# henriChevreux/distillation_trajectories

Measured on AMD Instinct MI355X. Metric: trajectory-timesteps/sec (B×T U-Net fwd) at 16×16 T=50, higher is better.
Workload: dtype f32 (fp32-accurate; convolutions: exact 3-plane bf16 operand split on bf16 MFMA with fp32 accumulate, or native fp32 MFMA, chosen per layer)

## Files before the change

### distillation_trajectories_amd/csrc/dt_conv_strip.hip

```cpp
#include <mutex>
#include <type_traits>

#include "dt_conv_epilogue.h"

namespace dt {

extern __shared__ __attribute__((aligned(16))) __bf16 strip_lds[];

template <int BM, int BN, int KC, int WK>
__global__ __launch_bounds__(256, find_strip_form(BM, BN, KC, WK)->waves_per_simd()) void conv_strip_bf16x6_kernel(const ConvParams p) {
  constexpr ConvForm F = *find_strip_form(BM, BN, KC, WK);
  constexpr int WN = F.wn(), WM = F.wm(), NT = 256;
  constexpr int MI = F.mi(), NI = F.ni();
  constexpr int KW = F.kw();
  static_assert(WM * WN * WK * 64 == NT && KC % WK == 0 && MI * 32 * WM == BM && NI * 32 * WN == BN && (WK == 1 || (MI == 2 && NI == 2)), "wave layout");
  constexpr int PLANE_B = F.plane_b(), STAGE_B = 3 * PLANE_B;
  constexpr int AP = F.ap();
  static_assert(2 * (BM + 2 * (F.max_w() + 1)) <= AP * NT, "strip staging reach");
  const int halo = strip_halo(p.W, BM);
  const int R = F.strip_rows(halo);
  const int RZ = F.zero_row(R);
  const int PLANE_A = F.plane_a(RZ);
  __bf16 *As = strip_lds;
  __bf16 *Bs = strip_lds + F.strip_elems(PLANE_A);

  const int tid = threadIdx.x, lane = tid & 63;
  const int wave = __builtin_amdgcn_readfirstlane(tid >> 6);
  const int wk = wave % WK, wm = (wave / WK) / WN, wn = (wave / WK) % WN;
  const int half = lane >> 5, l31 = lane & 31;
  const int m0 = blockIdx.x * BM, n0 = blockIdx.y * BN;
  const int HW = p.H * p.W;
  const int CC = p.cin_p >> 4;

  bool s_in[AP], s_ok[AP], s_core[AP];
  int s_off[AP], s_off2[AP], s_offb[AP], s_lds[AP];
#pragma unroll
  for (int i = 0; i < AP; ++i) {
    const int item = tid + i * NT;
    const int srow = item >> 1, hh = item & 1;
    const int m = m0 - halo + srow;
    s_in[i] = item < 2 * R;
    s_ok[i] = s_in[i] && m >= 0 && m < p.M;
    s_core[i] = s_ok[i] && srow >= halo && srow < halo + BM;
    const int mm = s_ok[i] ? m : 0;
    s_off[i] = mm * p.cin_p + hh * 8;
    s_off2[i] = mm * p.cin2_p + hh * 8;
    s_offb[i] = mm * p.b_stride + hh * 8;
    s_lds[i] = srow * 16 + ((hh ^ ((srow >> 3) & 1)) << 3);
  }
  constexpr bool B_ALL = WK > 1 && BN * 4 == NT;
  constexpr int NB = B_ALL ? KC * 3 / 2 : KC * 3, SB = B_ALL ? 2 : 1;
  static_assert(!B_ALL || (KC * 3) % 2 == 0, "weight staging");
  const bool b_thread = B_ALL || tid < BN * 2;
  const int bt = B_ALL ? (tid & (BN * 2 - 1)) : tid, bsub = B_ALL ? tid / (BN * 2) : 0;
  const size_t w_plane = (size_t)p.n_p * 16;
  const __bf16 *wbase = reinterpret_cast<const __bf16 *>(p.w) + (size_t)n0 * 16 + bt * 8 + bsub * w_plane;
  const __bf16 *wbase2 = reinterpret_cast<const __bf16 *>(p.w2) + (size_t)n0 * 16 + bt * 8 + bsub * w_plane;
  const int b_lds = bsub * PLANE_B + bt * 8;

  int a_row[MI];
  unsigned a_mask[MI];
#pragma unroll
  for (int mi = 0; mi < MI; ++mi) {
    const int row_i = wm * (MI * 32) + mi * 32 + l31;
    const int m = m0 + row_i;
    a_row[mi] = row_i + halo;
    unsigned mask = 0;
    if (m < p.M) {
      const int rem = m % HW;
      const int y = rem / p.W, x = rem - y * p.W;
#pragma unroll
      for (int t = 0; t < 9; ++t) {
        const int yy = y + t / 3 - 1, xx = x + t % 3 - 1;
        if (yy >= 0 && yy < p.H && xx >= 0 && xx < p.W) mask |= 1u << t;
      }
    }
    a_mask[mi] = mask;
  }
  int b_frag[NI];
#pragma unroll
  for (int ni = 0; ni < NI; ++ni) {
    const int row = wn * (NI * 32) + ni * 32 + l31;
    b_frag[ni] = row * 16 + ((half ^ ((row >> 3) & 1)) << 3);
  }

  f32x16 acc[MI][NI];
#pragma unroll
  for (int mi = 0; mi < MI; ++mi)
#pragma unroll
    for (int ni = 0; ni < NI; ++ni)
#pragma unroll
      for (int r = 0; r < 16; ++r) acc[mi][ni][r] = 0.f;

  const int n_main = (CC + p.splits * KC - 1) / (p.splits * KC);
  const int cc0 = blockIdx.z * n_main * KC;
  const int CC2 = p.cin2_p >> 4;
  const int n_chunks = n_main + (p.in2 ? (CC2 + KC - 1) / KC : 0);

  f32x4 sa0[KC][AP], sa1[KC][AP];
  u32x4 rb[NB];
  auto load_strip = [&](int ch) __attribute__((always_inline)) {
#pragma unroll
    for (int kk = 0; kk < KC; ++kk)
#pragma unroll
    for (int i = 0; i < AP; ++i) {
      sa0[kk][i] = f32x4{0.f, 0.f, 0.f, 0.f}; sa1[kk][i] = sa0[kk][i];
      if (ch < n_main) {
        const int cc = cc0 + ch * KC + kk;
        if (s_ok[i] && cc < CC) {
          const float *src = (p.in_b && cc >= p.cc_a) ? p.in_b + s_offb[i] + (cc - p.cc_a) * 16 : p.in + s_off[i] + cc * 16;
          sa0[kk][i] = *reinterpret_cast<const f32x4 *>(src);
          sa1[kk][i] = *reinterpret_cast<const f32x4 *>(src + 4);
        }
      } else if (s_core[i] && (ch - n_main) * KC + kk < CC2) {
        const int c2 = (ch - n_main) * KC + kk;
        const float *src = (p.in2_b && c2 >= p.cc_a) ? p.in2_b + s_offb[i] + (c2 - p.cc_a) * 16 : p.in2 + s_off2[i] + c2 * 16;
        sa0[kk][i] = *reinterpret_cast<const f32x4 *>(src);
        sa1[kk][i] = *reinterpret_cast<const f32x4 *>(src + 4);
      }
    }
  };
  auto write_strip = [&]() __attribute__((always_inline)) {
#pragma unroll
    for (int kk = 0; kk < KC; ++kk)
#pragma unroll
    for (int i = 0; i < AP; ++i)
      if (s_in[i]) {
        bf16x8 p1, p2, p3;
        split8(sa0[kk][i], sa1[kk][i], p1, p2, p3);
        __bf16 *A = As + kk * 3 * PLANE_A;
        *reinterpret_cast<bf16x8 *>(A + s_lds[i]) = p1;
        *reinterpret_cast<bf16x8 *>(A + PLANE_A + s_lds[i]) = p2;
        *reinterpret_cast<bf16x8 *>(A + 2 * PLANE_A + s_lds[i]) = p3;
      }
  };
  const size_t tap_stride = (size_t)p.ccw * 3 * w_plane, group_stride = (size_t)KC * 3 * w_plane;
  const __bf16 *wrun = wbase + (size_t)cc0 * 3 * w_plane;
  enum { ADV_NONE = 0, ADV_TAP, ADV_GROUP, ADV_SKIP0, ADV_SKIP };
  auto load_b = [&](int adv) __attribute__((always_inline)) {
    if (adv == ADV_TAP) wrun += tap_stride;
    else if (adv == ADV_GROUP) wrun = wrun - 8 * tap_stride + group_stride;
    else if (adv == ADV_SKIP0) wrun = wbase2;
    else if (adv == ADV_SKIP) wrun += group_stride;
    if (b_thread) {
#pragma unroll
      for (int i = 0; i < NB; ++i)
        rb[i] = *reinterpret_cast<const u32x4 *>(wrun + (SB * i) * w_plane);
    }
  };
  auto write_b = [&](int stage) __attribute__((always_inline)) {
    if (b_thread) {
      __bf16 *B = Bs + stage * KC * STAGE_B;
#pragma unroll
      for (int i = 0; i < NB; ++i) *reinterpret_cast<u32x4 *>(B + (SB * i) * PLANE_B + b_lds) = rb[i];
    }
  };

  constexpr bool DB = WK > 1;
  bf16x8 fbn[KW][NI][3];
  auto load_bd = [&](int adv) __attribute__((always_inline)) {
    if (adv == ADV_TAP) wrun += tap_stride;
    else if (adv == ADV_GROUP) wrun = wrun - 8 * tap_stride + group_stride;
    else if (adv == ADV_SKIP0) wrun = wbase2;
    else if (adv == ADV_SKIP) wrun += group_stride;
    const __bf16 *wt = wrun - (bt * 8 + bsub * w_plane);
#pragma unroll
    for (int kw = 0; kw < KW; ++kw)
#pragma unroll
      for (int ni = 0; ni < NI; ++ni)
#pragma unroll
        for (int pl = 0; pl < 3; ++pl)
          fbn[kw][ni][pl] = *reinterpret_cast<const bf16x8 *>(wt + ((wk * KW + kw) * 3 + pl) * w_plane + b_frag[ni]);
  };

  load_strip(0);
  if (DB) load_bd(ADV_NONE); else load_b(ADV_NONE);
  if (tid < 48 * KC) *reinterpret_cast<u32x4 *>(As + (tid >> 4) * PLANE_A + RZ * 16 + (tid & 15) * 8) = u32x4{0u, 0u, 0u, 0u};
  write_strip();
  if (!DB) write_b(0);
  __syncthreads();

  int step = 0;
  bool stage_next_strip = true;
  auto do_step = [&](auto TT, int ch, bool first_tap, bool last_tap, bool next_chunk, int adv) __attribute__((always_inline)) {
    constexpr int tt = decltype(TT)::value;
    const bool more = !last_tap || next_chunk;
    if (first_tap && next_chunk && stage_next_strip) load_strip(ch + 1);
    bf16x8 fbc[KW][NI][3];
    if (DB) {
#pragma unroll
      for (int kw = 0; kw < KW; ++kw)
#pragma unroll
        for (int ni = 0; ni < NI; ++ni)
#pragma unroll
          for (int pl = 0; pl < 3; ++pl) fbc[kw][ni][pl] = fbn[kw][ni][pl];
      if (more) load_bd(adv);
    } else if (more) load_b(adv);
    {
      int wv = p.W;
      asm volatile("" : "+s"(wv));
      const int shift = (tt / 3 - 1) * wv + (tt % 3 - 1);
      int a_e[MI];
#pragma unroll
      for (int mi = 0; mi < MI; ++mi) {
        int row0 = a_row[mi];
        asm volatile("" : "+v"(row0));
        const int srow = row0 + shift;
        const int lrow = ((a_mask[mi] >> tt) & 1u) ? srow : RZ + (srow & 7);
        a_e[mi] = lrow * 16 + ((half ^ ((srow >> 3) & 1)) << 3);
      }
#pragma unroll
      for (int kw = 0; kw < KW; ++kw) {
        const int kk = wk * KW + kw;
        const __bf16 *A = As + kk * 3 * PLANE_A;
        const __bf16 *B = Bs + ((step & 1) * KC + kk) * STAGE_B;
        bf16x8 fb[NI][3];
#pragma unroll
        for (int ni = 0; ni < NI; ++ni)
#pragma unroll
          for (int pl = 0; pl < 3; ++pl)
            fb[ni][pl] = DB ? fbc[kw][ni][pl] : *reinterpret_cast<const bf16x8 *>(B + pl * PLANE_B + b_frag[ni]);
#pragma unroll
        for (int mi = 0; mi < MI; ++mi) {
          bf16x8 fa[3];
#pragma unroll
          for (int pl = 0; pl < 3; ++pl)
            fa[pl] = *reinterpret_cast<const bf16x8 *>(A + pl * PLANE_A + a_e[mi]);
#pragma unroll
          for (int ni = 0; ni < NI; ++ni) mfma_bf16x6(acc[mi][ni], fa, fb[ni]);
        }
      }
    }
    if (!DB && more) write_b((step + 1) & 1);
    const bool restage = last_tap && next_chunk && stage_next_strip;
    if (restage) {
      __syncthreads();
      write_strip();
    }
    if (!DB || restage) __syncthreads();
    ++step;
  };

  constexpr bool DIRECT = MI * KW <= 2 && KC >= 2;
  f32x4 ga0[KW][MI][2], ga1[KW][MI][2];
  const int n_skip = p.in2 ? (CC2 + KC - 1) / KC : 0;
  auto load_a = [&](f32x4 (&g)[KW][MI][2], int s2) __attribute__((always_inline)) {
#pragma unroll
    for (int kw = 0; kw < KW; ++kw)
#pragma unroll
      for (int mi = 0; mi < MI; ++mi) {
        const int c2 = s2 * KC + wk * KW + kw;
        const int m = m0 + wm * (MI * 32) + mi * 32 + l31;
        g[kw][mi][0] = f32x4{0.f, 0.f, 0.f, 0.f}; g[kw][mi][1] = g[kw][mi][0];
        if (m < p.M && c2 < CC2) {
          const float *src = (p.in2_b && c2 >= p.cc_a) ? p.in2_b + (size_t)m * p.b_stride + (c2 - p.cc_a) * 16 + half * 8
                                                       : p.in2 + (size_t)m * p.cin2_p + c2 * 16 + half * 8;
          g[kw][mi][0] = *reinterpret_cast<const f32x4 *>(src);
          g[kw][mi][1] = *reinterpret_cast<const f32x4 *>(src + 4);
        }
      }
  };
  auto skip_step = [&](f32x4 (&g)[KW][MI][2], int s2) __attribute__((always_inline)) {
    const bool more = s2 + 1 < n_skip;
    bf16x8 fbc[KW][NI][3];
    if (DB) {
#pragma unroll
      for (int kw = 0; kw < KW; ++kw)
#pragma unroll
        for (int ni = 0; ni < NI; ++ni)
#pragma unroll
          for (int pl = 0; pl < 3; ++pl) fbc[kw][ni][pl] = fbn[kw][ni][pl];
      if (more) load_bd(ADV_SKIP);
    } else if (more) load_b(ADV_SKIP);
#pragma unroll
    for (int kw = 0; kw < KW; ++kw) {
      const int kk = wk * KW + kw;
      const __bf16 *B = Bs + ((step & 1) * KC + kk) * STAGE_B;
      bf16x8 fb[NI][3];
#pragma unroll
      for (int ni = 0; ni < NI; ++ni)
#pragma unroll
        for (int pl = 0; pl < 3; ++pl) fb[ni][pl] = DB ? fbc[kw][ni][pl] : *reinterpret_cast<const bf16x8 *>(B + pl * PLANE_B + b_frag[ni]);
#pragma unroll
      for (int mi = 0; mi < MI; ++mi) {
        bf16x8 fa[3];
        split8(g[kw][mi][0], g[kw][mi][1], fa[0], fa[1], fa[2]);
#pragma unroll
        for (int ni = 0; ni < NI; ++ni) mfma_bf16x6(acc[mi][ni], fa, fb[ni]);
      }
    }
    if (s2 + 2 < n_skip) load_a(g, s2 + 2);
    if (!DB) {
      if (more) write_b((step + 1) & 1);
      __syncthreads();
    }
    ++step;
  };

  const int prio_grp = ((blockIdx.x + gridDim.x * (blockIdx.y + gridDim.y * blockIdx.z)) >> 8) & 1;
  const bool use_prio = gridDim.x * gridDim.y * gridDim.z <= 512;
  for (int ch = 0; ch < n_main; ++ch) {
    if (use_prio) {
      if ((ch ^ prio_grp) & 1) __builtin_amdgcn_s_setprio(1);
      else __builtin_amdgcn_s_setprio(0);
    }
    const bool next_chunk = ch + 1 < ((WK > 1 && p.in2) ? n_main : n_chunks);
    if (DIRECT && WK == 1 && p.in2 && ch + 1 == n_main) {
      stage_next_strip = false;
      load_a(ga0, 0);
      if (n_skip > 1) load_a(ga1, 1);
    }
    do_step(std::integral_constant<int, 0>{}, ch, true, false, next_chunk, ADV_TAP);
    do_step(std::integral_constant<int, 1>{}, ch, false, false, next_chunk, ADV_TAP);
    do_step(std::integral_constant<int, 2>{}, ch, false, false, next_chunk, ADV_TAP);
    do_step(std::integral_constant<int, 3>{}, ch, false, false, next_chunk, ADV_TAP);
    do_step(std::integral_constant<int, 4>{}, ch, false, false, next_chunk, ADV_TAP);
    do_step(std::integral_constant<int, 5>{}, ch, false, false, next_chunk, ADV_TAP);
    do_step(std::integral_constant<int, 6>{}, ch, false, false, next_chunk, ADV_TAP);
    do_step(std::integral_constant<int, 7>{}, ch, false, false, next_chunk, ADV_TAP);
    do_step(std::integral_constant<int, 8>{}, ch, false, true, next_chunk, ch + 1 < n_main ? ADV_GROUP : ADV_SKIP0);
    if constexpr (WK == 1) {
      if (ch + 1 == n_main && p.in2) conv_midpoint<MI, NI>(p, acc, n0, wn, l31);
    }
  }
  if constexpr (WK > 1) {
    if (p.in2) {
      constexpr int P = F.pitch(), COPY = F.copy_floats();
      float *red = reinterpret_cast<float *>(strip_lds);
#pragma unroll
      for (int mi = 0; mi < MI; ++mi) {
        if (mi || DB) __syncthreads();
#pragma unroll
        for (int ni = 0; ni < NI; ++ni)
#pragma unroll
          for (int r = 0; r < 16; ++r)
            red[wk * COPY + (wm * 32 + 4 * half + (r & 3) + 8 * (r >> 2)) * P + wn * (NI * 32) + ni * 32 + l31] = acc[mi][ni][r];
        __syncthreads();
#pragma unroll
        for (int ni = 0; ni < NI; ++ni)
#pragma unroll
          for (int r = 0; r < 16; ++r) {
            const float *src = red + (wm * 32 + 4 * half + (r & 3) + 8 * (r >> 2)) * P + wn * (NI * 32) + ni * 32 + l31;
            float v = src[0];
#pragma unroll
            for (int c = 1; c < WK; ++c) v += src[c * COPY];
            acc[mi][ni][r] = wk == 0 ? v : 0.f;
          }
      }
      if (wk == 0) conv_midpoint<MI, NI>(p, acc, n0, wn, l31);
      __syncthreads();
      if (DB) load_bd(ADV_SKIP0); else load_b(ADV_SKIP0);
      if (DIRECT) {
        load_a(ga0, 0);
        if (n_skip > 1) load_a(ga1, 1);
      } else {
        load_strip(n_main);
        if (tid < 48 * KC) *reinterpret_cast<u32x4 *>(As + (tid >> 4) * PLANE_A + RZ * 16 + (tid & 15) * 8) = u32x4{0u, 0u, 0u, 0u};
        write_strip();
      }
      if (!DB) write_b(step & 1);
      __syncthreads();
    }
  }
  __builtin_amdgcn_s_setprio(0);
  if (DIRECT) {
    for (int s2 = 0; s2 < n_skip; s2 += 2) {
      skip_step(ga0, s2);
      if (s2 + 1 < n_skip) skip_step(ga1, s2 + 1);
    }
  } else {
    for (int ch = n_main; ch < n_chunks; ++ch)
      do_step(std::integral_constant<int, 4>{}, ch, true, true, ch + 1 < n_chunks, ADV_SKIP);
  }
  conv_epilogue<BM, BN, WK>(p, acc, reinterpret_cast<float *>(strip_lds), m0, n0, wm, wn, half, l31, wk);
}

#define DT_STRIP_ROW(cls, kind, bm, bn, kc, wk) {{kind, bm, bn, kc, wk, cls}, conv_strip_bf16x6_kernel<bm, bn, kc, wk>},
static const ConvKernel kStripKernels[] = {DT_CONV_FORMS_ALL_STRIP(DT_STRIP_ROW)};

static int strip_lds_attribute() {
  constexpr int kMaxDevices = 64;
  static std::mutex mu;
  static int status[kMaxDevices];
  int dev = 0;
  DT_HIP_TRY(hipGetDevice(&dev));
  if (dev < 0 || dev >= kMaxDevices) return DT_E_ARG;
  std::lock_guard<std::mutex> lock(mu);
  if (status[dev] == 0) {
    status[dev] = 1;
    for (const ConvKernel &k : kStripKernels) {
      if (!k.form.needs_lds_attribute()) continue;
      const hipError_t e = hipFuncSetAttribute(reinterpret_cast<const void *>(k.fn), hipFuncAttributeMaxDynamicSharedMemorySize, (int)k.form.lds_limit());
      if (e != hipSuccess) status[dev] = -(int)e;
    }
  }
  return status[dev] == 1 ? DT_OK : -status[dev];
}

int launch_conv_strip(const ConvParams &p_in, hipStream_t s) {
  ConvParams p = p_in;
  const ConvKernel &k = conv_kernel_of(kStripKernels, p);
  size_t lds = k.form.lds_bytes(p.W);
  p.dup_stage2 = p.n_dup == 2 && p.pool_out && k.form.dup_stage_bytes() <= k.form.lds_limit();
  if (p.dup_stage2 && k.form.dup_stage_bytes() > lds) lds = k.form.dup_stage_bytes();
  if (const int st = k.form.needs_lds_attribute() ? strip_lds_attribute() : DT_OK) return st;
  k.fn<<<dim3((p.M + p.bm - 1) / p.bm, p.n_p / p.bn, p.splits), 256, lds, s>>>(p);
  DT_LAUNCH_CHECK();
  return DT_OK;
}

}
```

Before: 349,000.

## Slim strip-kernel staging state and defer skip-input params to kernarg reload

Replaces the per-slot arrays of flags and three precomputed offsets with a single clamped row index plus an LDS slot that is -1 for inactive slots. Main and skip inputs become descriptor structs passed to one generic strip loader. The final main chunk is peeled out of the loop so the skip-path handling no longer needs runtime branches inside it. Skip-input parameters and the second weight base are re-read from the kernarg segment only after the main loop, to shorten their live ranges and cut register pressure. In exchange, offsets are recomputed with a multiply on every load, and skip strips now also load halo rows that are never used.

```diff
diff --git a/distillation_trajectories_amd/csrc/dt_conv_strip.hip b/distillation_trajectories_amd/csrc/dt_conv_strip.hip
--- a/distillation_trajectories_amd/csrc/dt_conv_strip.hip
+++ b/distillation_trajectories_amd/csrc/dt_conv_strip.hip
@@ -32,21 +32,15 @@
   const int HW = p.H * p.W;
   const int CC = p.cin_p >> 4;
 
-  bool s_in[AP], s_ok[AP], s_core[AP];
-  int s_off[AP], s_off2[AP], s_offb[AP], s_lds[AP];
+  const int s_h8 = (tid & 1) * 8;
+  int s_m[AP], s_lds[AP];
 #pragma unroll
   for (int i = 0; i < AP; ++i) {
     const int item = tid + i * NT;
     const int srow = item >> 1, hh = item & 1;
     const int m = m0 - halo + srow;
-    s_in[i] = item < 2 * R;
-    s_ok[i] = s_in[i] && m >= 0 && m < p.M;
-    s_core[i] = s_ok[i] && srow >= halo && srow < halo + BM;
-    const int mm = s_ok[i] ? m : 0;
-    s_off[i] = mm * p.cin_p + hh * 8;
-    s_off2[i] = mm * p.cin2_p + hh * 8;
-    s_offb[i] = mm * p.b_stride + hh * 8;
-    s_lds[i] = srow * 16 + ((hh ^ ((srow >> 3) & 1)) << 3);
+    s_m[i] = (item < 2 * R && m >= 0 && m < p.M) ? m : 0;
+    s_lds[i] = item < 2 * R ? srow * 16 + ((hh ^ ((srow >> 3) & 1)) << 3) : -1;
   }
   constexpr bool B_ALL = WK > 1 && BN * 4 == NT;
   constexpr int NB = B_ALL ? KC * 3 / 2 : KC * 3, SB = B_ALL ? 2 : 1;
@@ -55,7 +49,7 @@
   const int bt = B_ALL ? (tid & (BN * 2 - 1)) : tid, bsub = B_ALL ? tid / (BN * 2) : 0;
   const size_t w_plane = (size_t)p.n_p * 16;
   const __bf16 *wbase = reinterpret_cast<const __bf16 *>(p.w) + (size_t)n0 * 16 + bt * 8 + bsub * w_plane;
-  const __bf16 *wbase2 = reinterpret_cast<const __bf16 *>(p.w2) + (size_t)n0 * 16 + bt * 8 + bsub * w_plane;
+  const __bf16 *wbase2 = nullptr;
   const int b_lds = bsub * PLANE_B + bt * 8;
 
   int a_row[MI];
@@ -94,45 +88,49 @@
 
   const int n_main = (CC + p.splits * KC - 1) / (p.splits * KC);
   const int cc0 = blockIdx.z * n_main * KC;
-  const int CC2 = p.cin2_p >> 4;
-  const int n_chunks = n_main + (p.in2 ? (CC2 + KC - 1) / KC : 0);
+  const bool has_skip = p.in2 != nullptr;
+
+  struct StripSrc { const float *a, *b; int stride_a, stride_b, cc_split, cc_n; };
+  const StripSrc main_src = {p.in, p.in_b, p.cin_p, p.b_stride, p.in_b ? p.cc_a : CC, CC};
+  StripSrc skip_src = {};
 
   f32x4 sa0[KC][AP], sa1[KC][AP];
   u32x4 rb[NB];
-  auto load_strip = [&](int ch) __attribute__((always_inline)) {
+  auto load_strip = [&](const StripSrc &src, int c0) __attribute__((always_inline)) {
+#pragma unroll
+    for (int kk = 0; kk < KC; ++kk) {
+      const int cc = c0 + kk;
+      const bool live = cc < src.cc_n;
+      const bool from_b = cc >= src.cc_split;
+      const float *base = from_b ? src.b + (cc - src.cc_split) * 16 : src.a + cc * 16;
+      const int stride = from_b ? src.stride_b : src.stride_a;
+#pragma unroll
+      for (int i = 0; i < AP; ++i) {
+        sa0[kk][i] = f32x4{0.f, 0.f, 0.f, 0.f}; sa1[kk][i] = sa0[kk][i];
+        if (live) {
+          const float *s = base + (s_m[i] * stride + s_h8);
+          sa0[kk][i] = *reinterpret_cast<const f32x4 *>(s);
+          sa1[kk][i] = *reinterpret_cast<const f32x4 *>(s + 4);
+        }
+      }
+    }
+  };
+  auto write_strip = [&]() __attribute__((always_inline)) {
 #pragma unroll
     for (int kk = 0; kk < KC; ++kk)
 #pragma unroll
     for (int i = 0; i < AP; ++i) {
-      sa0[kk][i] = f32x4{0.f, 0.f, 0.f, 0.f}; sa1[kk][i] = sa0[kk][i];
-      if (ch < n_main) {
-        const int cc = cc0 + ch * KC + kk;
-        if (s_ok[i] && cc < CC) {
-          const float *src = (p.in_b && cc >= p.cc_a) ? p.in_b + s_offb[i] + (cc - p.cc_a) * 16 : p.in + s_off[i] + cc * 16;
-          sa0[kk][i] = *reinterpret_cast<const f32x4 *>(src);
-          sa1[kk][i] = *reinterpret_cast<const f32x4 *>(src + 4);
-        }
-      } else if (s_core[i] && (ch - n_main) * KC + kk < CC2) {
-        const int c2 = (ch - n_main) * KC + kk;
-        const float *src = (p.in2_b && c2 >= p.cc_a) ? p.in2_b + s_offb[i] + (c2 - p.cc_a) * 16 : p.in2 + s_off2[i] + c2 * 16;
-        sa0[kk][i] = *reinterpret_cast<const f32x4 *>(src);
-        sa1[kk][i] = *reinterpret_cast<const f32x4 *>(src + 4);
-      }
-    }
-  };
-  auto write_strip = [&]() __attribute__((always_inline)) {
-#pragma unroll
-    for (int kk = 0; kk < KC; ++kk)
-#pragma unroll
-    for (int i = 0; i < AP; ++i)
-      if (s_in[i]) {
+      int slot = s_lds[i];
+      asm volatile("" : "+v"(slot));
+      if (slot >= 0) {
         bf16x8 p1, p2, p3;
         split8(sa0[kk][i], sa1[kk][i], p1, p2, p3);
         __bf16 *A = As + kk * 3 * PLANE_A;
-        *reinterpret_cast<bf16x8 *>(A + s_lds[i]) = p1;
-        *reinterpret_cast<bf16x8 *>(A + PLANE_A + s_lds[i]) = p2;
-        *reinterpret_cast<bf16x8 *>(A + 2 * PLANE_A + s_lds[i]) = p3;
-      }
+        *reinterpret_cast<bf16x8 *>(A + slot) = p1;
+        *reinterpret_cast<bf16x8 *>(A + PLANE_A + slot) = p2;
+        *reinterpret_cast<bf16x8 *>(A + 2 * PLANE_A + slot) = p3;
+      }
+    }
   };
   const size_t tap_stride = (size_t)p.ccw * 3 * w_plane, group_stride = (size_t)KC * 3 * w_plane;
   const __bf16 *wrun = wbase + (size_t)cc0 * 3 * w_plane;
@@ -173,7 +171,7 @@
           fbn[kw][ni][pl] = *reinterpret_cast<const bf16x8 *>(wt + ((wk * KW + kw) * 3 + pl) * w_plane + b_frag[ni]);
   };
 
-  load_strip(0);
+  load_strip(main_src, cc0);
   if (DB) load_bd(ADV_NONE); else load_b(ADV_NONE);
   if (tid < 48 * KC) *reinterpret_cast<u32x4 *>(As + (tid >> 4) * PLANE_A + RZ * 16 + (tid & 15) * 8) = u32x4{0u, 0u, 0u, 0u};
   write_strip();
@@ -181,11 +179,11 @@
   __syncthreads();
 
   int step = 0;
-  bool stage_next_strip = true;
-  auto do_step = [&](auto TT, int ch, bool first_tap, bool last_tap, bool next_chunk, int adv) __attribute__((always_inline)) {
+  auto do_step = [&](auto TT, bool first_tap, bool last_tap, bool next_chunk, int adv, const StripSrc &next, int c_next,
+                     bool stage_next) __attribute__((always_inline)) {
     constexpr int tt = decltype(TT)::value;
     const bool more = !last_tap || next_chunk;
-    if (first_tap && next_chunk && stage_next_strip) load_strip(ch + 1);
+    if (first_tap && next_chunk && stage_next) load_strip(next, c_next);
     bf16x8 fbc[KW][NI][3];
     if (DB) {
 #pragma unroll
@@ -232,7 +230,7 @@
       }
     }
     if (!DB && more) write_b((step + 1) & 1);
-    const bool restage = last_tap && next_chunk && stage_next_strip;
+    const bool restage = last_tap && next_chunk && stage_next;
     if (restage) {
       __syncthreads();
       write_strip();
@@ -241,9 +239,43 @@
     ++step;
   };
 
+  const int prio_grp = ((blockIdx.x + gridDim.x * (blockIdx.y + gridDim.y * blockIdx.z)) >> 8) & 1;
+  const bool use_prio = gridDim.x * gridDim.y * gridDim.z <= 512;
+  auto chunk_group = [&](int ch, bool next_chunk, int adv_last, const StripSrc &next, int c_next, bool stage_next) __attribute__((always_inline)) {
+    if (use_prio) {
+      if ((ch ^ prio_grp) & 1) __builtin_amdgcn_s_setprio(1);
+      else __builtin_amdgcn_s_setprio(0);
+    }
+    do_step(std::integral_constant<int, 0>{}, true, false, next_chunk, ADV_TAP, next, c_next, stage_next);
+    do_step(std::integral_constant<int, 1>{}, false, false, next_chunk, ADV_TAP, next, c_next, stage_next);
+    do_step(std::integral_constant<int, 2>{}, false, false, next_chunk, ADV_TAP, next, c_next, stage_next);
+    do_step(std::integral_constant<int, 3>{}, false, false, next_chunk, ADV_TAP, next, c_next, stage_next);
+    do_step(std::integral_constant<int, 4>{}, false, false, next_chunk, ADV_TAP, next, c_next, stage_next);
+    do_step(std::integral_constant<int, 5>{}, false, false, next_chunk, ADV_TAP, next, c_next, stage_next);
+    do_step(std::integral_constant<int, 6>{}, false, false, next_chunk, ADV_TAP, next, c_next, stage_next);
+    do_step(std::integral_constant<int, 7>{}, false, false, next_chunk, ADV_TAP, next, c_next, stage_next);
+    do_step(std::integral_constant<int, 8>{}, false, true, next_chunk, adv_last, next, c_next, stage_next);
+  };
+  const int n_loop = (WK == 1 && has_skip) ? n_main - 1 : n_main;
+  for (int ch = 0; ch < n_loop; ++ch)
+    chunk_group(ch, ch + 1 < n_main, ADV_GROUP, main_src, cc0 + (ch + 1) * KC, true);
+
+  typedef const __attribute__((address_space(4))) ConvParams KernargParams;
+  KernargParams *qp = (KernargParams *)__builtin_amdgcn_kernarg_segment_ptr();
+  asm volatile("" : "+s"(qp));
+  const ConvParams q = *(const ConvParams *)qp;
+
   constexpr bool DIRECT = MI * KW <= 2 && KC >= 2;
   f32x4 ga0[KW][MI][2], ga1[KW][MI][2];
-  const int n_skip = p.in2 ? (CC2 + KC - 1) / KC : 0;
+  int n_skip = 0;
+  if (has_skip) {
+    const int CC2 = q.cin2_p >> 4;
+    skip_src = StripSrc{q.in2, q.in2_b, q.cin2_p, q.b_stride, q.in2_b ? q.cc_a : CC2, CC2};
+    n_skip = (CC2 + KC - 1) / KC;
+    wbase2 = reinterpret_cast<const __bf16 *>(q.w2) + (size_t)n0 * 16 + bt * 8 + bsub * w_plane;
+  }
+  const int n_chunks = n_main + n_skip;
+  const int M_rows = q.M;
   auto load_a = [&](f32x4 (&g)[KW][MI][2], int s2) __attribute__((always_inline)) {
 #pragma unroll
     for (int kw = 0; kw < KW; ++kw)
@@ -252,9 +284,9 @@
         const int c2 = s2 * KC + wk * KW + kw;
         const int m = m0 + wm * (MI * 32) + mi * 32 + l31;
         g[kw][mi][0] = f32x4{0.f, 0.f, 0.f, 0.f}; g[kw][mi][1] = g[kw][mi][0];
-        if (m < p.M && c2 < CC2) {
-          const float *src = (p.in2_b && c2 >= p.cc_a) ? p.in2_b + (size_t)m * p.b_stride + (c2 - p.cc_a) * 16 + half * 8
-                                                       : p.in2 + (size_t)m * p.cin2_p + c2 * 16 + half * 8;
+        if (m < M_rows && c2 < skip_src.cc_n) {
+          const float *src = c2 >= skip_src.cc_split ? skip_src.b + (size_t)m * skip_src.stride_b + (c2 - skip_src.cc_split) * 16 + half * 8
+                                                     : skip_src.a + (size_t)m * skip_src.stride_a + c2 * 16 + half * 8;
           g[kw][mi][0] = *reinterpret_cast<const f32x4 *>(src);
           g[kw][mi][1] = *reinterpret_cast<const f32x4 *>(src + 4);
         }
@@ -297,34 +329,18 @@
     ++step;
   };
 
-  const int prio_grp = ((blockIdx.x + gridDim.x * (blockIdx.y + gridDim.y * blockIdx.z)) >> 8) & 1;
-  const bool use_prio = gridDim.x * gridDim.y * gridDim.z <= 512;
-  for (int ch = 0; ch < n_main; ++ch) {
-    if (use_prio) {
-      if ((ch ^ prio_grp) & 1) __builtin_amdgcn_s_setprio(1);
-      else __builtin_amdgcn_s_setprio(0);
-    }
-    const bool next_chunk = ch + 1 < ((WK > 1 && p.in2) ? n_main : n_chunks);
-    if (DIRECT && WK == 1 && p.in2 && ch + 1 == n_main) {
-      stage_next_strip = false;
-      load_a(ga0, 0);
-      if (n_skip > 1) load_a(ga1, 1);
-    }
-    do_step(std::integral_constant<int, 0>{}, ch, true, false, next_chunk, ADV_TAP);
-    do_step(std::integral_constant<int, 1>{}, ch, false, false, next_chunk, ADV_TAP);
-    do_step(std::integral_constant<int, 2>{}, ch, false, false, next_chunk, ADV_TAP);
-    do_step(std::integral_constant<int, 3>{}, ch, false, false, next_chunk, ADV_TAP);
-    do_step(std::integral_constant<int, 4>{}, ch, false, false, next_chunk, ADV_TAP);
-    do_step(std::integral_constant<int, 5>{}, ch, false, false, next_chunk, ADV_TAP);
-    do_step(std::integral_constant<int, 6>{}, ch, false, false, next_chunk, ADV_TAP);
-    do_step(std::integral_constant<int, 7>{}, ch, false, false, next_chunk, ADV_TAP);
-    do_step(std::integral_constant<int, 8>{}, ch, false, true, next_chunk, ch + 1 < n_main ? ADV_GROUP : ADV_SKIP0);
-    if constexpr (WK == 1) {
-      if (ch + 1 == n_main && p.in2) conv_midpoint<MI, NI>(p, acc, n0, wn, l31);
+  if constexpr (WK == 1) {
+    if (has_skip) {
+      if (DIRECT) {
+        load_a(ga0, 0);
+        if (n_skip > 1) load_a(ga1, 1);
+      }
+      chunk_group(n_main - 1, n_main < n_chunks, ADV_SKIP0, skip_src, 0, !DIRECT);
+      conv_midpoint<MI, NI>(q, acc, n0, wn, l31);
     }
   }
   if constexpr (WK > 1) {
-    if (p.in2) {
+    if (has_skip) {
       constexpr int P = F.pitch(), COPY = F.copy_floats();
       float *red = reinterpret_cast<float *>(strip_lds);
 #pragma unroll
@@ -347,14 +363,14 @@
             acc[mi][ni][r] = wk == 0 ? v : 0.f;
           }
       }
-      if (wk == 0) conv_midpoint<MI, NI>(p, acc, n0, wn, l31);
+      if (wk == 0) conv_midpoint<MI, NI>(q, acc, n0, wn, l31);
       __syncthreads();
       if (DB) load_bd(ADV_SKIP0); else load_b(ADV_SKIP0);
       if (DIRECT) {
         load_a(ga0, 0);
         if (n_skip > 1) load_a(ga1, 1);
       } else {
-        load_strip(n_main);
+        load_strip(skip_src, 0);
         if (tid < 48 * KC) *reinterpret_cast<u32x4 *>(As + (tid >> 4) * PLANE_A + RZ * 16 + (tid & 15) * 8) = u32x4{0u, 0u, 0u, 0u};
         write_strip();
       }
@@ -370,9 +386,9 @@
     }
   } else {
     for (int ch = n_main; ch < n_chunks; ++ch)
-      do_step(std::integral_constant<int, 4>{}, ch, true, true, ch + 1 < n_chunks, ADV_SKIP);
-  }
-  conv_epilogue<BM, BN, WK>(p, acc, reinterpret_cast<float *>(strip_lds), m0, n0, wm, wn, half, l31, wk);
+      do_step(std::integral_constant<int, 4>{}, true, true, ch + 1 < n_chunks, ADV_SKIP, skip_src, (ch + 1 - n_main) * KC, true);
+  }
+  conv_epilogue<BM, BN, WK>(q, acc, reinterpret_cast<float *>(strip_lds), m0, n0, wm, wn, half, l31, wk);
 }
 
 #define DT_STRIP_ROW(cls, kind, bm, bn, kc, wk) {{kind, bm, bn, kc, wk, cls}, conv_strip_bf16x6_kernel<bm, bn, kc, wk>},
```

Result: slower. 344,700 (-1.2%).
